# stgl/scarplet

Hardware: AMD Instinct MI355X
Metric: Mpixel·template/s (DEM pixels × ages × orientations / s) (higher is better)
Workload: dtype f32

## Files before the change

scarplet_amd/csrc/sc_api.hip:

```cpp
#include "sc_internal.h"
#include <stdarg.h>
#include <stdio.h>
#include <string.h>
#include <stdlib.h>
#include <math.h>
#include <algorithm>

int sc_fail(sc_ctx* ctx, int code, const char* fmt, ...) {
    char buf[1024];
    va_list ap;
    va_start(ap, fmt);
    vsnprintf(buf, sizeof(buf), fmt, ap);
    va_end(ap);
    if (ctx) ctx->err = buf;
    return code;
}

int sc_ensure(sc_ctx* ctx, DevBuf& b, size_t bytes) {
    if (bytes <= b.cap && b.p) return SC_OK;
    if (b.p) {
        SC_HIP(ctx, hipFree(b.p));
        b.p = nullptr;
        b.cap = 0;
    }
    if (bytes == 0) bytes = 16;
    SC_HIP(ctx, hipMalloc(&b.p, bytes));
    b.cap = bytes;
    return SC_OK;
}

static void buf_free(DevBuf& b) {
    if (b.p) (void)hipFree(b.p);
    b.p = nullptr;
    b.cap = 0;
}

size_t sc_total_bytes(sc_ctx* c) {
    DevBuf* arr[] = {&c->z, &c->xaxis, &c->yaxis, &c->A, &c->B, &c->C, &c->curv,
                     &c->best_snr, &c->best_amp, &c->best_id, &c->map_amp,
                     &c->map_snr, &c->templ, &c->sums, &c->wl1, &c->norms, &c->norm_part, &c->win_w, &c->win_m,
                     &c->tw_y, &c->tw_x, &c->blk, &c->uc, &c->uc2, &c->vh, &c->wh, &c->mh,
                     &c->yw, &c->ym, &c->tiles, &c->halo_z, &c->halo_stage, &c->res, &c->sib_buf, &c->dwin, &c->spans, &c->res_stats, &c->digest, &c->split_s, &c->split_a, &c->split_i,
                     &c->near, &c->near_ev, &c->score, &c->score_w, &c->score_abc, &c->st_slot, &c->st_work, &c->st_pairs, &c->st_patch, &c->st_spans, &c->snap, &c->xch, &c->xch_cnt,
                     &c->tr_planes, &c->tr_thin, &c->tr_par, &c->tr_lab, &c->tr_cnt, &c->tr_bsum, &c->tr_tot, &c->tr_sort, &c->tr_hist, &c->tr_rbsum, &c->tr_seg};
    size_t s = 0;
    for (DevBuf* b : arr) s += b->cap;
    for (auto& w : c->windows) s += (size_t)w.h * w.wd * 13;
    return s;
}

int sc_lds_attr(sc_ctx* ctx, const void* kernel, size_t bytes) {
    auto it = ctx->lds_attr.find(kernel);
    if (it != ctx->lds_attr.end() && it->second >= bytes) return SC_OK;
    SC_HIP(ctx, hipFuncSetAttribute(kernel, hipFuncAttributeMaxDynamicSharedMemorySize,
                                    (int)bytes));
    ctx->lds_attr[kernel] = bytes;
    return SC_OK;
}

void sc_prof_begin(sc_ctx* ctx, int kernel) {
    ctx->prof_cur = -1;
    ctx->prof_kernel = kernel;
    const long long b = ctx->k_brackets[kernel]++;
    if (!ctx->prof) return;
// ... 84 lines not shown
        if (!(value >= 0.0)) return sc_fail(ctx, SC_ERR_INVALID, "batch_fill must be >= 0");
        ctx->batch_fill = (int)value;
    } else if (!strcmp(name, "i1_pairs")) {
        if (!(value >= 1.0 && value <= 64.0)) return sc_fail(ctx, SC_ERR_INVALID, "i1_pairs must be 1 .. 64");
        ctx->i1_pairs = (int)value;
    } else if (!strcmp(name, "near_window")) {
        if (!(value >= 0.0 && value < 1.0)) return sc_fail(ctx, SC_ERR_INVALID, "near_window must be in [0, 1)");
        ctx->near_w = (float)value;
    } else if (!strcmp(name, "batch_templ")) {
        if (!(value >= 0.0 && value <= (double)SC_MAX_BATCH)) return sc_fail(ctx, SC_ERR_INVALID, "batch_templ must be 0 .. %d", SC_MAX_BATCH);
        ctx->batch_templ = (int)value;
    } else if (!strcmp(name, "split_i1")) {
        if (!(value >= 0.0 && value <= 64.0)) return sc_fail(ctx, SC_ERR_INVALID, "split_i1 must be 0 .. 64");
        ctx->split_i1 = (int)value;
    } else if (!strcmp(name, "split_fill")) {
        if (!(value >= 0.0)) return sc_fail(ctx, SC_ERR_INVALID, "split_fill must be >= 0");
        ctx->split_fill = (long long)value;
    } else if (!strcmp(name, "sib")) {
        ctx->sib = (int)value;
    } else if (!strcmp(name, "spectra_mb")) {
        if (!(value >= 0.0)) return sc_fail(ctx, SC_ERR_INVALID, "spectra_mb must be >= 0");
        ctx->spec_mb = value;
        fft_spectra_forget(ctx);
    } else if (!strcmp(name, "y_gb")) {
        if (!(value >= 0.0)) return sc_fail(ctx, SC_ERR_INVALID, "y_gb must be >= 0");
        ctx->y_gb = value;
    } else {
        return sc_fail(ctx, SC_ERR_INVALID, "unknown option '%s'", name);
    }
    return SC_OK;
}

extern "C" int sc_clear_windows(sc_ctx* ctx) {
    if (!ctx) return SC_ERR_INVALID;
    (void)hipStreamSynchronize(ctx->stream);
    for (auto& w : ctx->windows) {
        if (w.w) (void)hipFree(w.w);
        if (w.w64) (void)hipFree(w.w64);
        if (w.m) (void)hipFree(w.m);
        if (w.mask_lim) (void)hipFree(w.mask_lim);
        if (w.mask_err) (void)hipFree(w.mask_err);
    }
    ctx->windows.clear();
    return SC_OK;
}

extern "C" void sc_destroy(sc_ctx* c) {
    if (!c) return;
    (void)hipSetDevice(c->device);
    (void)hipStreamSynchronize(c->stream);
    sc_comm_destroy(c);
    sc_prof_collect(c);
    for (auto& e : c->ev_pool) {
        (void)hipEventDestroy(e.first);
        (void)hipEventDestroy(e.second);
    }
    sc_clear_windows(c);
    DevBuf* arr[] = {&c->z, &c->xaxis, &c->yaxis, &c->A, &c->B, &c->C, &c->curv,
                     &c->best_snr, &c->best_amp, &c->best_id, &c->map_amp,
                     &c->map_snr, &c->templ, &c->sums, &c->wl1, &c->norms, &c->norm_part, &c->win_w, &c->win_m,
                     &c->tw_y, &c->tw_x, &c->blk, &c->uc, &c->uc2, &c->vh, &c->wh, &c->mh,
                     &c->yw, &c->ym, &c->tiles, &c->halo_z, &c->halo_stage, &c->res, &c->sib_buf, &c->dwin, &c->spans, &c->res_stats, &c->digest, &c->split_s, &c->split_a, &c->split_i,
                     &c->near, &c->near_ev, &c->score, &c->score_w, &c->score_abc, &c->st_slot, &c->st_work, &c->st_pairs, &c->st_patch, &c->st_spans, &c->snap, &c->xch, &c->xch_cnt,
                     &c->tr_planes, &c->tr_thin, &c->tr_par, &c->tr_lab, &c->tr_cnt, &c->tr_bsum, &c->tr_tot, &c->tr_sort, &c->tr_hist, &c->tr_rbsum, &c->tr_seg};
    for (DevBuf* b : arr) buf_free(*b);
    for (int k = 0; k < 4; ++k) buf_free(c->cmp[k]);
    for (int k = 0; k < 4; ++k) buf_free(c->cmp_in[k]);
    for (int k = 0; k < 4; ++k) buf_free(c->fill[k]);
    (void)hipStreamDestroy(c->stream);
    delete c;
}

extern "C" const char* sc_last_error(sc_ctx* ctx) {
    return ctx ? ctx->err.c_str() : "null context";
}

extern "C" size_t sc_device_bytes(sc_ctx* ctx) { return ctx ? sc_total_bytes(ctx) : 0; }

static int set_dem_body(sc_ctx* ctx, int ly, int lx, int gy0, int gx0, int ny,
                        int nx, int cy0, int cy1, int cx0, int cx1, double dx,
                        double dy, int wrap, const double* xaxis,
                        const double* yaxis);

static int set_dem_common(sc_ctx* ctx, int ly, int lx, int gy0, int gx0, int ny,
// ... 843 lines not shown
```

scarplet_amd/csrc/sc_fft.hip:

```cpp
#include "sc_internal.h"
#include <math.h>
#include <type_traits>
#include <string.h>

struct TileDev {
    int i0, j0, vy, vx, gi0, gj0;
};

#ifndef SC_I1_XLANE
#define SC_I1_XLANE 1
#endif
#ifndef SC_I2_RD1
#define SC_I2_RD1 1
#endif
#ifndef SC_LDS_WR1
#define SC_LDS_WR1 0
#endif
#ifndef SC_LDS_RD1
#define SC_LDS_RD1 1
#endif
#ifndef SC_H2_XLANE
#define SC_H2_XLANE 1
#endif
#ifndef SC_F1C_HOLD
// ... 1203 lines not shown
    if constexpr (!XP) TAKE_TEMPLATE_SHARE(PT, (size_t)TY * Tx)
    if ((j >> 3) & 1)
        inv_cols_sym_body<TY, true, PT, XP>((Tx >> 2) - 1 - i, uc, uc2, wa, mb, Tx, 0, pair, vfirst, G, rp_lo, rp_hi, phx,
                                            parity, tw, yw, ym, ystride, dbg, np, pcj, tstride, tiles, py_valid);
    else
        inv_cols_sym_body<TY, false, PT, XP>(i, uc, uc2, wa, mb, Tx, 0, pair, vfirst, G, rp_lo, rp_hi, phx,
                                             parity, tw, yw, ym, ystride, dbg, np, pcj, tstride, tiles, py_valid);
}

template <int TY>
__host__ __device__ constexpr int w8_line() { return TY + TY / 16 + 4; }
template <int TY>
__host__ __device__ constexpr size_t w8_lds() {
    return ((size_t)8 * w8_line<TY>() + (SC_I1_TWTAB ? 16 : 4) * (TY / 16 + TY / 256) + SC_MAX_GROUP) * sizeof(float2);
}

template <int TY, bool MIRROR, bool PT, int NC>
__device__ __forceinline__ void
inv_cols_w8_body(const int B, const int jobx, const float2* __restrict__ uc, const float2* __restrict__ uc2,
                 const float* __restrict__ wa, const float* __restrict__ mb, int Tx,
                 int pair, int vfirst, int G, int rp_lo, int rp_hi, const float2* __restrict__ phx,
                 int parity, const float2* __restrict__ tw, float2* __restrict__ yw,
                 float2* __restrict__ ym, int ystride, int np, int pcj, int tstride,
                 const TileDev* __restrict__ tiles, int py_valid, const TemplDev* __restrict__ tl) {
    extern __shared__ __attribute__((aligned(16))) float2 sm[];
    constexpr int S = TY / 16;
    static_assert(S % 64 == 0 && S / 64 <= 2, "one wave per line: 64 or 128 sets");
    constexpr int U = S / 64;
    constexpr int NK = 16 * U;
    constexpr int LINE = w8_line<TY>();
    const int w = __builtin_amdgcn_readfirstlane(threadIdx.x >> 6), lane = threadIdx.x & 63;
    float2* line = sm + w * LINE;
    int i0A = 0, i0B = 0, vyA = 0, vyB = 0;
    {
        const int ob = jobx / pcj, q = jobx - ob * pcj;
        const TileDev tA_ = tiles[2 * (pair + q)], tB_ = tiles[2 * (pair + q) + 1];
        i0A = tA_.i0; i0B = tB_.i0; vyA = tA_.vy; vyB = tB_.vy;
        if (py_valid >= 0) {
            const int vy = max(tA_.vy, tB_.vy);
            rp_hi = min(rp_hi, (py_valid + vy - 1) >> 1);
        }
        pair += ob * np + q;
        vfirst += ob * tstride;
    }
    int2* const rng = reinterpret_cast<int2*>(sm + NC * LINE + (SC_I1_TWTAB ? 16 : 4) * (S + S / 16));
    {
        const int NGt = PT ? (G + 1) / 2 : G;
// ... 33 lines not shown
        float2* t = st2 ? t2 + (i - S) : t1 + i;
        const float2 wb[4] = {tw[e], tw[2 * e], tw[4 * e], tw[8 * e]};
        pk::v2 wk[16];
        twiddle16_expand(wb, wk);
#pragma unroll
        for (int k = 1; k < 16; ++k) t[k * n] = make_float2(wk[k].x, wk[k].y);
    }
#else
    float2* t2 = t1 + 4 * S;
    for (int i = threadIdx.x; i < 4 * S; i += 64 * NC) t1[i] = tw[(i % S) << (i / S)];
    for (int i = threadIdx.x; i < 4 * (S / 16); i += 64 * NC) t2[i] = tw[((i % (S / 16)) << 4) << (i / (S / 16))];
#endif
    auto tw_of = [&](const float2* t, int n, int idx, float2 (&wq)[4]) {
#pragma unroll
        for (int m = 0; m < 4; ++m) wq[m] = lds_cell<true>(t + m * n + idx);
    };
    float c[NK], c2[PT ? NK : 1];
    const int NG = PT ? (G + 1) / 2 : G;
    for (int pl = 0; pl < 2; ++pl) {
        const float2* xcol = (pl ? uc2 : uc) + (size_t)pair * plane + (size_t)ft * TY;
        const float* hsrc = (pl ? mb : wa) + (size_t)vfirst * hplane + (size_t)fs * TY;
        const bool rot = pl == 0 && parity == 1;
        float2 xp[NK];
#pragma unroll
        for (int k = 0; k < NK; ++k) {
            const int fy = lane + 64 * k;
            float2 pv;
            if (!MIRROR) {
                pv = phase_tab(tw + TY, phx, fy, ft);
            } else {
                pv = phase_tab(tw + TY, phx, (TY - fy) & (TY - 1), (Tx - ft) & (Tx - 1));
                pv.y = -pv.y;
            }
            float2 v = cmul(xcol[fy], pv);
            if (rot) v = MIRROR ? make_float2(v.y, -v.x) : make_float2(-v.y, v.x);
            xp[k] = v;
        }
        const float* cbase = hsrc + (MIRROR ? TY - lane : lane);
        const int c0off = (MIRROR && lane == 0) ? -TY : 0;
        auto fetch = [&](int gi_, int u) {
            const float* p = cbase + (size_t)(PT ? 2 * gi_ : gi_) * hplane;
            const bool has2 = PT && 2 * gi_ + 1 < G;
            const float* p2 = has2 ? p + hplane : p;
            const unsigned keep2 = has2 ? ~0u : 0u;
#pragma unroll
            for (int k = 0; k < NK; ++k) {
                if (u >= 0 && k % U != u) continue;
                const int off = k ? (MIRROR ? -64 * k : 64 * k) : c0off;
                c[k] = p[off];
                if constexpr (PT) c2[k] = __uint_as_float(__float_as_uint(p2[off]) & keep2);
            }
        };
        fetch(0, -1);
        for (int gi_ = 0; gi_ < NG; ++gi_) {
            lds_barrier();
            float2 wq[4];
            int lt = lane;
            asm volatile("" : "+v"(lt));
#pragma unroll
// ... 90 lines not shown
                    __builtin_nontemporal_store(f2{c0.x, c0.y}, reinterpret_cast<f2*>(p));
                    __builtin_nontemporal_store(f2{c1.x, c1.y}, reinterpret_cast<f2*>(p + Tx));
                }
            } else
#endif
#pragma unroll 2
            for (int rp = s_lo + RQ * w + ln / NC; rp <= s_hi; rp += RQ * NC)
                store_stream(o + (size_t)rp * (Tx >> 3) * 16, lds_cell<true>(lc + ph(2 * rp)), lds_cell<true>(lc + ph(2 * rp + 1)));
#ifdef SC_I1_PRIO
            __builtin_amdgcn_s_setprio(0);
#endif
        }
        lds_barrier();
    }
}

template <int TY, bool PT>
__global__ void __launch_bounds__(512, (TY == 1024 && !PT) ? 4 : 2)
k_inv_cols_w8(const float2* __restrict__ uc, const float2* __restrict__ uc2,
              const float* __restrict__ wa, const float* __restrict__ mb, int Tx,
              int pair, int vfirst, int G, int rp_lo, int rp_hi, const float2* __restrict__ phx,
              int parity, const float2* __restrict__ tw, float2* __restrict__ yw,
              float2* __restrict__ ym, int ystride, int np, int pcj, int tstride,
              const TileDev* __restrict__ tiles, int py_valid, const TemplDev* __restrict__ tl, int jil) {
    const int L = blockIdx.x, g16 = L / (16 * jil), r16 = L - g16 * 16 * jil, jq = r16 >> 4, j = r16 & 15;
    const int i = (g16 << 3) | (j & 7), jobx = (int)blockIdx.y * jil + jq;
    TAKE_TEMPLATE_SHARE(PT, (size_t)TY * Tx)
    if ((j >> 3) & 1)
        inv_cols_w8_body<TY, true, PT, 8>((Tx >> 3) - 1 - i, jobx, uc, uc2, wa, mb, Tx, pair, vfirst, G, rp_lo,
                                   rp_hi, phx, parity, tw, yw, ym, ystride, np, pcj, tstride, tiles, py_valid, tl);
    else
        inv_cols_w8_body<TY, false, PT, 8>(i, jobx, uc, uc2, wa, mb, Tx, pair, vfirst, G, rp_lo,
                                    rp_hi, phx, parity, tw, yw, ym, ystride, np, pcj, tstride, tiles, py_valid, tl);
}

template <int TY, bool PT>
__global__ void __launch_bounds__(256, 1)
k_inv_cols_w4(const float2* __restrict__ uc, const float2* __restrict__ uc2,
              const float* __restrict__ wa, const float* __restrict__ mb, int Tx,
              int pair, int vfirst, int G, int rp_lo, int rp_hi, const float2* __restrict__ phx,
              int parity, const float2* __restrict__ tw, float2* __restrict__ yw,
              float2* __restrict__ ym, int ystride, int np, int pcj, int tstride,
              const TileDev* __restrict__ tiles, int py_valid, const TemplDev* __restrict__ tl) {
    const int j = blockIdx.x, i = ((j >> 4) << 3) | (j & 7);
    if ((j >> 3) & 1)
        inv_cols_w8_body<TY, true, PT, 4>((Tx >> 2) - 1 - i, (int)blockIdx.y, uc, uc2, wa, mb, Tx, pair, vfirst, G, rp_lo,
                                          rp_hi, phx, parity, tw, yw, ym, ystride, np, pcj, tstride, tiles, py_valid, tl);
    else
        inv_cols_w8_body<TY, false, PT, 4>(i, (int)blockIdx.y, uc, uc2, wa, mb, Tx, pair, vfirst, G, rp_lo,
                                           rp_hi, phx, parity, tw, yw, ym, ystride, np, pcj, tstride, tiles, py_valid, tl);
}

constexpr int H2_TY = 512, H2_COLS = 16;
__host__ __device__ constexpr size_t h2_lds() {
    return ((size_t)H2_COLS * w8_line<H2_TY>() + 4 * (H2_TY / 16 + H2_TY / 256) + SC_MAX_GROUP) * sizeof(float2);
}
template <bool MIRROR, bool PT, bool XP>
__device__ __forceinline__ void
inv_cols_h2_body(const int B, const int jobx, const float2* __restrict__ uc, const float2* __restrict__ uc2,
                 const float* __restrict__ wa, const float* __restrict__ mb, int Tx,
                 int pair, int vfirst, int G, int rp_lo, int rp_hi, const float2* __restrict__ phx,
                 int parity, const float2* __restrict__ tw, float2* __restrict__ yw,
                 float2* __restrict__ ym, int ystride, int np, int pcj, int tstride,
                 const TileDev* __restrict__ tiles, int py_valid, const TemplDev* __restrict__ tl) {
    extern __shared__ __attribute__((aligned(16))) float2 sm[];
    constexpr int TY = H2_TY, S = TY / 16, NK = 16, NC = H2_COLS;
    constexpr int LINE = w8_line<TY>();
    static_assert(S == 32 && !(XP && !PT), "half a wave per column; paired orientations are a paired-template mode");
    const int w = __builtin_amdgcn_readfirstlane(threadIdx.x >> 6), lane = threadIdx.x & 63;
    const int hl = lane & 31, cw = 2 * w + (lane >> 5);
    float2* line = sm + cw * LINE;
    int i0A = 0, i0B = 0, vyA = 0, vyB = 0, pairB = 0;
    if constexpr (XP) {
// ... 1003 lines not shown
}

static int upload_twiddles(sc_ctx* ctx, DevBuf& buf, int& have, int T, int kph) {
    const int key = T * 8 + (kph & 7);
    if (have == key) return SC_OK;
    std::vector<float2> h(2 * (size_t)T);
    for (int k = 0; k < T; ++k) {
        double a = -2.0 * M_PI * (double)k / (double)T;
        h[k] = make_float2((float)cos(a), (float)sin(a));
        long long m = ((long long)kph * k) % (2LL * T);
        double b = M_PI * (double)m / (double)T;
        h[T + k] = make_float2((float)cos(b), (float)sin(b));
    }
    int rc = sc_ensure(ctx, buf, sizeof(float2) * h.size());
    if (rc) return rc;
    SC_HIP(ctx, hipStreamSynchronize(ctx->stream));
    SC_HIP(ctx, hipMemcpy(buf.p, h.data(), sizeof(float2) * h.size(), hipMemcpyHostToDevice));
    have = key;
    return SC_OK;
}

static int npairs_of(const FftGeom& fg) { return (fg.ntiles + 1) / 2; }

void fft_spectra_forget(sc_ctx* ctx) {
    std::fill(ctx->spec_key.begin(), ctx->spec_key.end(), NAN);
}

int fft_prepare(sc_ctx* ctx, const FftGeom& fg, int n_templ_chunk, int group, int nb, int n_slots) {
    if (!fft_size_supported(fg.Ty) || !fft_size_supported(fg.Tx))
        return sc_fail(ctx, SC_ERR_UNSUPPORTED, "FFT tile %dx%d not supported", fg.Ty, fg.Tx);
    int rc;
    if ((rc = upload_twiddles(ctx, ctx->tw_y, ctx->tw_Ty, fg.Ty, 1 - ctx->g.oy))) return rc;
    if ((rc = upload_twiddles(ctx, ctx->tw_x, ctx->tw_Tx, fg.Tx, 1 - ctx->g.ox))) return rc;
    const Geom& g = ctx->g;
    int np = npairs_of(fg);
    std::vector<TileDev> h(2 * np);
    for (int k = 0; k < 2 * np; ++k) {
        TileDev t{0, 0, 0, 0, 0, 0};
        if (k < fg.ntiles) {
            int ty = k / fg.ntx, tx = k % fg.ntx;
            t.i0 = g.cy0 + ty * fg.Vy;
            t.j0 = g.cx0 + tx * fg.Vx;
            t.vy = std::min(fg.Vy, g.cy1 - t.i0);
            t.vx = std::min(fg.Vx, g.cx1 - t.j0);
            t.gi0 = t.i0 + g.oy - fg.Py;
            t.gj0 = t.j0 + g.ox - fg.Qx;
// ... 17 lines not shown
        const Geom& gg = ctx->g;
        const long long sig[24] = {fg.Ty, fg.Tx, fg.Vy, fg.Vx, fg.nty, fg.ntx, fg.circ_y, fg.circ_x, fg.Py, fg.Qx,
                                   gg.ly, gg.lx, gg.gy0, gg.gx0, gg.ny, gg.nx, gg.cy0, gg.cy1, gg.cx0, gg.cx1,
                                   gg.wrap, n_slots, 0, 0};
        bool keep = n_slots > 0 && 2.0 * (double)plane * np * n_slots <= ctx->spec_mb * 1048576.0;
        if (keep) {
            const double add = 2.0 * (double)plane * np * n_slots - (double)(ctx->uc.cap + ctx->uc2.cap);
            size_t free_b = 0, total_b = 0;
            if (add > 0.0 && (hipMemGetInfo(&free_b, &total_b) != hipSuccess || add > 0.25 * (double)free_b))
                keep = false;
        }
        const int slots = keep ? n_slots : 0;
        const size_t have = std::max(nb, slots);
        if (ctx->uc.cap > 2 * plane * np * have + ((size_t)256 << 20)) {
            SC_HIP(ctx, hipStreamSynchronize(ctx->stream));
            for (DevBuf* b : {&ctx->uc, &ctx->uc2}) {
                if (b->p) SC_HIP(ctx, hipFree(b->p));
                b->p = nullptr;
                b->cap = 0;
            }
        }
        const void *p0 = ctx->uc.p, *p1 = ctx->uc2.p, *p2 = ctx->norms.p;
        if ((rc = sc_ensure(ctx, ctx->norms, sizeof(double) * 2 * np * have))) return rc;
        if ((rc = sc_ensure(ctx, ctx->uc, plane * np * have))) return rc;
        if ((rc = sc_ensure(ctx, ctx->uc2, plane * np * have))) return rc;
        if (!keep || slots != ctx->spec_slots || memcmp(sig, ctx->spec_sig, sizeof(sig)) != 0 ||
            p0 != ctx->uc.p || p1 != ctx->uc2.p || p2 != ctx->norms.p) {
            ctx->spec_key.assign((size_t)3 * slots, NAN);
            memcpy(ctx->spec_sig, sig, sizeof(sig));
        }
        ctx->spec_slots = slots;
        ctx->spec_uc_stride = (size_t)np * fg.Ty * fg.Tx;
        ctx->spec_norm_stride = (size_t)2 * np;
        ctx->uc_off = ctx->norms_off = 0;
    }
    if ((rc = sc_ensure(ctx, ctx->norm_part, sizeof(double) * 2 * np * nb * (fg.Ty / 4)))) return rc;
    if ((rc = sc_ensure(ctx, ctx->curv, sizeof(float) * (size_t)ctx->g.ly * ctx->g.lx * nb))) return rc;
    if ((rc = sc_ensure(ctx, ctx->vh, plane * n_templ_chunk))) return rc;
    size_t hplane = half_plane(fg.Ty, fg.Tx) * sizeof(float2);
    if ((rc = sc_ensure(ctx, ctx->wh, hplane * n_templ_chunk))) return rc;
    if ((rc = sc_ensure(ctx, ctx->mh, hplane * n_templ_chunk))) return rc;
    int pb = 1;
    {
        size_t free_b = 0, total_b = 0;
        double budget = 0.0;
        if (hipMemGetInfo(&free_b, &total_b) == hipSuccess)
            budget = std::min(32e9, 0.25 * (double)(free_b + ctx->yw.cap + ctx->ym.cap));
        if (ctx->y_gb > 0.0) budget = ctx->y_gb * 1e9;
// ... 27 lines not shown
    }
    out.slots = (uint32_t*)ctx->sib_buf.p;
    out.base = (++ctx->sib_epoch) << 8;
    return SC_OK;
}

template <typename K>
static int set_lds(sc_ctx* ctx, K kernel, size_t bytes) {
    return sc_lds_attr(ctx, (const void*)kernel, bytes);
}

#define DISPATCH_T(T, FN)                                                     \
    switch (T) {                                                              \
        case 64: FN(64); break;                                               \
        case 128: FN(128); break;                                             \
        case 256: FN(256); break;                                             \
        case 512: FN(512); break;                                             \
        case 1024: FN(1024); break;                                           \
        case 2048: FN(2048); break;                                           \
        case 4096: FN(4096); break;                                           \
        default: return sc_fail(ctx, SC_ERR_UNSUPPORTED, "tile size %d", T);  \
    }

static int launch_fwd_cols(sc_ctx* ctx, const FftGeom& fg, int nplanes,
                           float2* out0, float2* out1, int split2,
                           const TemplDev* templ = nullptr) {
    size_t lds = fft_lds_bytes(fg.Ty);
    dim3 grid(fg.Tx / 4, nplanes);
    sc_prof_begin(ctx, SC_K_FWD_COLS);
#define FN(T)                                                                  \
    {                                                                          \
        int rc = set_lds(ctx, k_fwd_cols<T>, lds);                             \
        if (rc) return rc;                                                     \
        hipLaunchKernelGGL(k_fwd_cols<T>, grid, dim3(fft_threads(T)), lds,     \
                           ctx->stream, (const float2*)ctx->blk.p, fg.Tx,      \
                           (const float2*)ctx->tw_y.p, out0, out1, split2,     \
                           templ);                                             \
    }
    DISPATCH_T(fg.Ty, FN)
#undef FN
    sc_prof_end(ctx);
    SC_HIP(ctx, hipGetLastError());
    return SC_OK;
}

int fft_forward_curv(sc_ctx* ctx, const FftGeom& fg, int nb, const float (*coef)[3]) {
    int np = npairs_of(fg);
    size_t lds = fft_lds_bytes(fg.Tx);
    dim3 grid(fg.Ty / 4 / FWD_ROWS_RBW, np * nb);
    CurvMix mixc;
    memset(&mixc, 0, sizeof(mixc));
    if (coef) {
        if (nb > SC_MAX_ORIENT) return sc_fail(ctx, SC_ERR_INVALID, "curvature batch of %d planes", nb);
        for (int b = 0; b < nb; ++b)
            for (int j = 0; j < 3; ++j) mixc.c[b][j] = coef[b][j];
    }
    sc_prof_begin(ctx, SC_K_FWD_ROWS);
#define FN2(T, MIXV)                                                           \
    {                                                                          \
        int rc = set_lds(ctx, k_fwd_rows_curv<T, MIXV>, lds);                  \
        if (rc) return rc;                                                     \
        hipLaunchKernelGGL((k_fwd_rows_curv<T, MIXV>), grid, dim3(fft_threads(T)), \
                           lds, ctx->stream, (const float*)(MIXV ? ctx->A.p : ctx->curv.p), \
                           (const float*)ctx->B.p, (const float*)ctx->C.p, mixc, \
                           ctx->g, (const TileDev*)ctx->tiles.p, fg.Ty,        \
                           (const float2*)ctx->tw_x.p, (float2*)ctx->blk.p,    \
                           (double*)ctx->norm_part.p, ctx->dbg, np,            \
                           (size_t)ctx->g.ly * ctx->g.lx);                     \
    }
#define FN(T) { if (coef) FN2(T, true) else FN2(T, false) }
    DISPATCH_T(fg.Tx, FN)
#undef FN
#undef FN2
    hipLaunchKernelGGL(k_tile_norms, dim3(np * nb), dim3(64), 0, ctx->stream,
                       (const double*)ctx->norm_part.p, fg.Ty / 4, (double*)ctx->norms.p + ctx->norms_off);
    sc_prof_end(ctx);
    SC_HIP(ctx, hipGetLastError());
    return launch_fwd_cols(ctx, fg, 2 * np * nb, (float2*)ctx->uc.p + ctx->uc_off, (float2*)ctx->uc2.p + ctx->uc_off, 1);
}

static bool fft_use_sym(const sc_ctx* ctx, const FftGeom& fg, int parity) {
    return parity != 0 && fg.Ty <= 2048 && ctx->variant != 8;
}

int fft_forward_templates(sc_ctx* ctx, const FftGeom& fg, int first, int n, int parity) {
    size_t lds = fft_lds_bytes(fg.Tx);
    dim3 grid(fg.Ty / 4, n);
    sc_prof_begin(ctx, SC_K_FWD_ROWS);
#define FN(T)                                                                  \
    {                                                                          \
        int rc = set_lds(ctx, k_fwd_rows_templ<T>, lds);                       \
        if (rc) return rc;                                                     \
        hipLaunchKernelGGL(k_fwd_rows_templ<T>, grid, dim3(fft_threads(T)),    \
                           lds, ctx->stream, (const TemplDev*)ctx->templ.p,    \
                           first, (const float*)ctx->win_w.p,                  \
                           (const uint8_t*)ctx->win_m.p,                       \
                           (const double*)ctx->sums.p, fg.Ty,                  \
                           (const float2*)ctx->tw_x.p, (float2*)ctx->blk.p);   \
    }
    DISPATCH_T(fg.Tx, FN)
#undef FN
// ... 5 lines not shown
        sc_prof_begin(ctx, SC_K_FWD_COLS);
#define FN(T)                                                                  \
    {                                                                          \
        int rc = set_lds(ctx, k_fwd_cols_tsym<T>, ldsc);                       \
        if (rc) return rc;                                                     \
        hipLaunchKernelGGL(k_fwd_cols_tsym<T>, gridc, dim3(fft_threads(T)), ldsc, ctx->stream, \
                           (const float2*)ctx->blk.p, fg.Tx, (const float2*)ctx->tw_y.p, \
                           (const TemplDev*)ctx->templ.p + first, (const float2*)ctx->tw_x.p + fg.Tx, \
                           parity, (float*)ctx->wh.p, (float*)ctx->mh.p);      \
    }
        switch (fg.Ty) {
            case 64: FN(64); break;
            case 128: FN(128); break;
            case 256: FN(256); break;
            case 512: FN(512); break;
            case 1024: FN(1024); break;
            default: FN(2048); break;
        }
#undef FN
        sc_prof_end(ctx);
        SC_HIP(ctx, hipGetLastError());
        return SC_OK;
    }
    int rc = launch_fwd_cols(ctx, fg, n, (float2*)ctx->vh.p, nullptr, 0,
                             (const TemplDev*)ctx->templ.p + first);
    if (rc) return rc;
    size_t cells = half_plane(fg.Ty, fg.Tx);
    dim3 grid_s((unsigned)((cells / 2 + 255) / 256), n);
    sc_prof_begin(ctx, SC_K_FWD_COLS);
    if (fft_use_sym(ctx, fg, parity))
        hipLaunchKernelGGL(k_split_templ_sym, grid_s, dim3(256), 0, ctx->stream,
                           (const float2*)ctx->vh.p, fg.Ty, fg.Tx, (const float2*)ctx->tw_y.p + fg.Ty,
                           (const float2*)ctx->tw_x.p + fg.Tx,
                           parity, (float*)ctx->wh.p, (float*)ctx->mh.p);
    else
        hipLaunchKernelGGL(k_split_templ, grid_s, dim3(256), 0, ctx->stream, (const float2*)ctx->vh.p,
                           fg.Ty, fg.Tx, (float2*)ctx->wh.p, (float2*)ctx->mh.p);
    sc_prof_end(ctx);
    SC_HIP(ctx, hipGetLastError());
    return SC_OK;
}

int fft_inverse_fold(sc_ctx* ctx, const FftGeom& fg, int first, int n,
                     int group, bool to_maps, bool full_masks, int parity, int nb) {
    const bool sym = fft_use_sym(ctx, fg, parity);
    int np = npairs_of(fg);
    size_t lds_r = fft_lds_bytes(fg.Tx);
    int rp_lo = 0, rp_hi = fg.Ty / 2 - 1;
    if (!fg.circ_y) {
        rp_lo = fg.Py / 2;
        rp_hi = std::min(fg.Ty - 1, fg.Py + fg.Vy - 1) / 2;
    }
    const int rp_n = rp_hi - rp_lo + 1;
    if (group > SC_MAX_GROUP)
        return sc_fail(ctx, SC_ERR_INVALID, "group %d exceeds %d", group, SC_MAX_GROUP);
    const int pb = std::max(1, ctx->fft_pb);
    const size_t yblock = (size_t)fg.Ty * fg.Tx * group;
    const bool fast = (fg.Tx == 512 || fg.Tx == 1024 || fg.Tx == 2048) && ctx->variant != 9;
    const bool symx = sym && ctx->variant != 6 && fg.Ty >= 512 && fg.Ty <= 2048 && (fg.Tx / 8) % 8 == 0;
    const bool w8 = symx && ctx->variant != 2 && (fg.Ty == 2048 || fg.Ty == 1024) && (fg.Tx / 16) % 8 == 0;
    if (nb > 1 && (!fast || n > group || nb * n > SC_MAX_BATCH || n > SC_MAX_GROUP))
        return sc_fail(ctx, SC_ERR_INVALID, "orientation batching outside its conditions");
    auto chunk = [&](int pair0, int pc, auto ptc) -> int {
        constexpr bool PTV = decltype(ptc)::value;
        for (int g0 = 0; g0 < n; g0 += group) {
            int G = std::min(group, n - g0);
            const bool xp = PTV && n == 1 && nb >= 2 && pc == 1 && sym && symx && fg.Ty == 512 &&
                            ctx->variant != 12 && !to_maps;
            const size_t lds_c = (size_t)4 * fft_line(fg.Ty) * sizeof(float2) +
                                 (fg.Ty <= 2048 ? (size_t)4 * fg.Ty * sizeof(float2) : 0);
            const int slots = 256 * (int)std::max<size_t>(1, (size_t)(160 * 1024) / lds_c);
            int pi1 = nb > 1 ? pc : std::max(1, std::min(pc, (slots + fg.Tx / 8 - 1) / (fg.Tx / 8)));
            int jil = 1;
            if (nb == 1 && w8 && (!PTV || fg.Ty == 1024) && ctx->variant != 1 && !xp && ctx->i1_pairs > 1) {
                jil = std::min(pc, ctx->i1_pairs);
                pi1 = jil;
            }
            const bool row_skip = !full_masks && !to_maps && ctx->variant != 13;
            auto parts_for = [&](long long workgroups, long long capacity, int transforms) {
                if (!ctx->split_i1 || workgroups <= 0) return 1;
                if (ctx->split_i1 > 1) return std::max(1, std::min(ctx->split_i1, transforms));
                int best = 1;
                double best_u = 0.0;
                for (int nz = 1; nz <= 8 && transforms / nz >= 4; ++nz) {
                    const long long w = workgroups * nz, rounds = (w + capacity - 1) / capacity;
// ... 20 lines not shown
    ctx->stream, (const float2*)ctx->uc.p + ctx->uc_off, (const float2*)ctx->uc2.p + ctx->uc_off, (const float*)ctx->wh.p, \
        (const float*)ctx->mh.p, fg.Tx, CB0, pair, g0, G, rp_lo, rp_hi,                    \
        (const float2*)ctx->tw_x.p + fg.Tx, parity, (const float2*)ctx->tw_y.p, ywp, ymp, group
#define SYM_ARGS_D(CB0) SYM_ARGS(CB0), ctx->dbg, np, pcc, n, (const TileDev*)ctx->tiles.p, fg.circ_y ? -1 : fg.Py
#define FN_SYMX(T)                                                             \
    {                                                                          \
        int rc = set_lds(ctx, k_inv_cols_symx<T, PTV>, inv_cols_lds<T>());     \
        if (rc) return rc;                                                     \
        const int nz_ = parts_for((long long)(fg.Tx / 4) * nb * pcc,                                \
                                  256LL * std::max<size_t>(1, std::min<size_t>((160 * 1024) / inv_cols_lds<T>(), \
                                                                               2048 / fft_threads(T) / 2)), NGl); \
        hipLaunchKernelGGL((k_inv_cols_symx<T, PTV>), dim3(fg.Tx / 4, nb * pcc, nz_), dim3(fft_threads(T)), \
                           inv_cols_lds<T>(), ctx->stream, (const float2*)ctx->uc.p + ctx->uc_off, (const float2*)ctx->uc2.p + ctx->uc_off, \
                           (const float*)ctx->wh.p, (const float*)ctx->mh.p, fg.Tx, pair, g0, G, rp_lo, rp_hi, \
                           (const float2*)ctx->tw_x.p + fg.Tx, parity, (const float2*)ctx->tw_y.p, ywp, ymp, group, \
                           ctx->dbg, np, pcc, n, (const TileDev*)ctx->tiles.p, fg.circ_y ? -1 : fg.Py); \
    }
#define FN_W8(T)                                                               \
    {                                                                          \
        int rc = set_lds(ctx, k_inv_cols_w8<T, PTV>, w8_lds<T>());             \
        if (rc) return rc;                                                     \
        const int nz_ = parts_for((long long)(fg.Tx / 8) * nb * pcc, 256LL * ((T == 1024 && !PTV) ? 2 : 1), NGl); \
        hipLaunchKernelGGL((k_inv_cols_w8<T, PTV>), dim3(fg.Tx / 8 * jilc, nb * pcc / jilc, nz_), dim3(512),  \
                           w8_lds<T>(), ctx->stream, (const float2*)ctx->uc.p + ctx->uc_off, (const float2*)ctx->uc2.p + ctx->uc_off, \
                           (const float*)ctx->wh.p, (const float*)ctx->mh.p, fg.Tx, pair, g0, G, rp_lo, rp_hi, \
                           (const float2*)ctx->tw_x.p + fg.Tx, parity, (const float2*)ctx->tw_y.p, ywp, ymp, group, \
                           np, pcc, n, (const TileDev*)ctx->tiles.p, fg.circ_y ? -1 : fg.Py, \
                           row_skip ? (const TemplDev*)ctx->templ.p + first : nullptr, jilc); \
    }
#define FN_W4(T)                                                               \
    {                                                                          \
         \
        const size_t lds4 = (size_t)88 * 1024;                                 \
        int rc = set_lds(ctx, k_inv_cols_w4<T, PTV>, lds4);                    \
        if (rc) return rc;                                                     \
        hipLaunchKernelGGL((k_inv_cols_w4<T, PTV>), dim3(fg.Tx / 4, nb * pcc), dim3(256),  \
                           lds4, ctx->stream, (const float2*)ctx->uc.p + ctx->uc_off, (const float2*)ctx->uc2.p + ctx->uc_off, \
                           (const float*)ctx->wh.p, (const float*)ctx->mh.p, fg.Tx, pair, g0, G, rp_lo, rp_hi, \
                           (const float2*)ctx->tw_x.p + fg.Tx, parity, (const float2*)ctx->tw_y.p, ywp, ymp, group, \
                           np, pcc, n, (const TileDev*)ctx->tiles.p, fg.circ_y ? -1 : fg.Py, \
                           row_skip ? (const TemplDev*)ctx->templ.p + first : nullptr); \
    }
#define FN_SYM(T)                                                              \
    {                                                                          \
        int rc = set_lds(ctx, k_inv_cols_sym<T, false, PTV>, inv_cols_lds<T>());    \
        if (rc) return rc;                                                     \
        rc = set_lds(ctx, k_inv_cols_sym<T, true, PTV>, inv_cols_lds<T>());         \
        if (rc) return rc;                                                     \
        const int nlo = fg.Tx / 8, nhi = fg.Tx / 4 - nlo;                      \
        hipLaunchKernelGGL((k_inv_cols_sym<T, false, PTV>), dim3(nlo, nb * pcc), dim3(fft_threads(T)), \
                           inv_cols_lds<T>(), SYM_ARGS_D(0));                  \
        if (nhi > 0)                                                           \
            hipLaunchKernelGGL((k_inv_cols_sym<T, true, PTV>), dim3(nhi, nb * pcc), dim3(fft_threads(T)), \
                               inv_cols_lds<T>(), SYM_ARGS_D(nlo));            \
    }
#define FN(T)                                                                  \
    {                                                                          \
        int rc = set_lds(ctx, k_inv_cols<T, false>, inv_cols_lds<T>());        \
        if (rc) return rc;                                                     \
        rc = set_lds(ctx, k_inv_cols<T, true>, inv_cols_lds<T>());             \
        if (rc) return rc;                                                     \
        const int nlo = fg.Tx / 8, nhi = fg.Tx / 4 - nlo;                      \
        hipLaunchKernelGGL((k_inv_cols<T, false>), dim3(nlo, nb * pcc), dim3(fft_threads(T)), \
                           inv_cols_lds<T>(), COL_ARGS(0));                    \
// ... 219 lines not shown
```

scarplet_amd/csrc/sc_internal.h:

```cpp
#pragma once
#include <hip/hip_runtime.h>
#include <stdint.h>
#include <string>
#include <vector>
#include <map>
#include <limits.h>
#include "../../include/scarplet_hip.h"

#define SC_EPS 2.220446049250313e-16
#define SC_EVENT_WORDS 4

#ifdef SC_ABLATE
#define SC_DBGBIT(d, b) (((d) & (b)) != 0)
#else
#define SC_DBGBIT(d, b) false
#endif
#define SC_EXP_UNDERFLOW 745.1332191019412

struct TemplDev {
    int32_t kind, flags;
    double cos_a, sin_a, c, d, p0, p1;
    int32_t ilo, ihi, jlo, jhi;
    int32_t pmin, pmax, qmin, qmax;
    uint32_t id;
// ... 52 lines not shown
    long long dem_nan = 0;
    double dem_sig[16] = {0};
    bool dem_unchanged = false;
    DevBuf digest;
    DevBuf best_snr, best_amp, best_id;
    DevBuf map_amp, map_snr;
    DevBuf cmp[4], cmp_in[4];
    size_t cmp_n = 0;
    DevBuf res_stats;
    DevBuf dwin, spans;
    DevBuf templ, sums, wl1, norms, win_w, win_m;
    DevBuf norm_part;
    double spec_mb = 0.0;
    int spec_slots = 0;
    size_t spec_uc_stride = 0;
    size_t spec_norm_stride = 0;
    size_t uc_off = 0, norms_off = 0;
    std::vector<double> spec_key;
    long long spec_sig[24] = {0};
    DevBuf tw_y, tw_x;
    int tw_Ty = 0, tw_Tx = 0;
    int fft_pb = 1;
    DevBuf blk, uc, uc2, vh, wh, mh, yw, ym, tiles;
    std::vector<WindowSlot> windows;
    std::vector<TemplDev> h_templ;
    std::vector<double> h_sums, h_wl1;
    std::vector<int> h_wslot;
    std::vector<double> h_mix;
    std::vector<unsigned char> h_tiles;
    bool async_in_flight = false;
    int last_batch = 0;
    float kappa = 4.f;
    float near_w = 0.f;
    float near_w_used = 0.f;
    DevBuf near;
    DevBuf near_ev;
    DevBuf st_slot, st_work, st_pairs, st_patch, st_spans;
    DevBuf snap;
    size_t snap_cells = 0;
    long long cand_n = -1;
    DevBuf xch, xch_cnt;
    long long xch_n = -1;
    size_t patch_n = 0;
    DevBuf score;
    DevBuf score_w;
    DevBuf score_abc;
// ... 191 lines not shown
```

Measured before the change: 192,700.

## Fuse forward column FFT of curvature spectra into w8 inverse column kernel

When enabled (default on) and spectra are not cached, the row-FFT output is kept in a new buffer and the forward column FFT is performed inside the w8 inverse-column kernel, loading from that buffer into LDS, instead of running a separate forward-column pass that writes uc/uc2. This removes one full kernel launch and a global round-trip of the spectra. The catch is that the forward column FFT is recomputed in every inverse-column launch (per template group), and the fused kernel carries more registers. A fallback materializes uc/uc2 when the fused path doesn't apply.

Result: faster. 197,400, median of 6 (+2.4%).

```diff
diff --git a/scarplet_amd/csrc/sc_api.hip b/scarplet_amd/csrc/sc_api.hip
--- a/scarplet_amd/csrc/sc_api.hip
+++ b/scarplet_amd/csrc/sc_api.hip
@@ -39,7 +39,7 @@
     DevBuf* arr[] = {&c->z, &c->xaxis, &c->yaxis, &c->A, &c->B, &c->C, &c->curv,
                      &c->best_snr, &c->best_amp, &c->best_id, &c->map_amp,
                      &c->map_snr, &c->templ, &c->sums, &c->wl1, &c->norms, &c->norm_part, &c->win_w, &c->win_m,
-                     &c->tw_y, &c->tw_x, &c->blk, &c->uc, &c->uc2, &c->vh, &c->wh, &c->mh,
+                     &c->tw_y, &c->tw_x, &c->blk, &c->cblk, &c->uc, &c->uc2, &c->vh, &c->wh, &c->mh,
                      &c->yw, &c->ym, &c->tiles, &c->halo_z, &c->halo_stage, &c->res, &c->sib_buf, &c->dwin, &c->spans, &c->res_stats, &c->digest, &c->split_s, &c->split_a, &c->split_i,
                      &c->near, &c->near_ev, &c->score, &c->score_w, &c->score_abc, &c->st_slot, &c->st_work, &c->st_pairs, &c->st_patch, &c->st_spans, &c->snap, &c->xch, &c->xch_cnt,
                      &c->tr_planes, &c->tr_thin, &c->tr_par, &c->tr_lab, &c->tr_cnt, &c->tr_bsum, &c->tr_tot, &c->tr_sort, &c->tr_hist, &c->tr_rbsum, &c->tr_seg};
@@ -170,6 +170,8 @@
         if (!(value >= 0.0)) return sc_fail(ctx, SC_ERR_INVALID, "spectra_mb must be >= 0");
         ctx->spec_mb = value;
         fft_spectra_forget(ctx);
+    } else if (!strcmp(name, "fuse_fwd")) {
+        ctx->fuse_fwd = value != 0.0;
     } else if (!strcmp(name, "y_gb")) {
         if (!(value >= 0.0)) return sc_fail(ctx, SC_ERR_INVALID, "y_gb must be >= 0");
         ctx->y_gb = value;
@@ -207,7 +209,7 @@
     DevBuf* arr[] = {&c->z, &c->xaxis, &c->yaxis, &c->A, &c->B, &c->C, &c->curv,
                      &c->best_snr, &c->best_amp, &c->best_id, &c->map_amp,
                      &c->map_snr, &c->templ, &c->sums, &c->wl1, &c->norms, &c->norm_part, &c->win_w, &c->win_m,
-                     &c->tw_y, &c->tw_x, &c->blk, &c->uc, &c->uc2, &c->vh, &c->wh, &c->mh,
+                     &c->tw_y, &c->tw_x, &c->blk, &c->cblk, &c->uc, &c->uc2, &c->vh, &c->wh, &c->mh,
                      &c->yw, &c->ym, &c->tiles, &c->halo_z, &c->halo_stage, &c->res, &c->sib_buf, &c->dwin, &c->spans, &c->res_stats, &c->digest, &c->split_s, &c->split_a, &c->split_i,
                      &c->near, &c->near_ev, &c->score, &c->score_w, &c->score_abc, &c->st_slot, &c->st_work, &c->st_pairs, &c->st_patch, &c->st_spans, &c->snap, &c->xch, &c->xch_cnt,
                      &c->tr_planes, &c->tr_thin, &c->tr_par, &c->tr_lab, &c->tr_cnt, &c->tr_bsum, &c->tr_tot, &c->tr_sort, &c->tr_hist, &c->tr_rbsum, &c->tr_seg};
diff --git a/scarplet_amd/csrc/sc_fft.hip b/scarplet_amd/csrc/sc_fft.hip
--- a/scarplet_amd/csrc/sc_fft.hip
+++ b/scarplet_amd/csrc/sc_fft.hip
@@ -1249,7 +1249,7 @@
                  int pair, int vfirst, int G, int rp_lo, int rp_hi, const float2* __restrict__ phx,
                  int parity, const float2* __restrict__ tw, float2* __restrict__ yw,
                  float2* __restrict__ ym, int ystride, int np, int pcj, int tstride,
-                 const TileDev* __restrict__ tiles, int py_valid, const TemplDev* __restrict__ tl) {
+                 const TileDev* __restrict__ tiles, int py_valid, const TemplDev* __restrict__ tl, const bool fwd) {
     extern __shared__ __attribute__((aligned(16))) float2 sm[];
     constexpr int S = TY / 16;
     static_assert(S % 64 == 0 && S / 64 <= 2, "one wave per line: 64 or 128 sets");
@@ -1329,19 +1329,108 @@
         const float* hsrc = (pl ? mb : wa) + (size_t)vfirst * hplane + (size_t)fs * TY;
         const bool rot = pl == 0 && parity == 1;
         float2 xp[NK];
-#pragma unroll
-        for (int k = 0; k < NK; ++k) {
-            const int fy = lane + 64 * k;
-            float2 pv;
-            if (!MIRROR) {
-                pv = phase_tab(tw + TY, phx, fy, ft);
+        auto park = [&](auto get) {
+#pragma unroll
+            for (int k = 0; k < NK; ++k) {
+                const int fy = lane + 64 * k;
+                float2 pv;
+                if (!MIRROR) {
+                    pv = phase_tab(tw + TY, phx, fy, ft);
+                } else {
+                    pv = phase_tab(tw + TY, phx, (TY - fy) & (TY - 1), (Tx - ft) & (Tx - 1));
+                    pv.y = -pv.y;
+                }
+                float2 v = cmul(get(k), pv);
+                if (rot) v = MIRROR ? make_float2(v.y, -v.x) : make_float2(-v.y, v.x);
+                xp[k] = v;
+            }
+        };
+        if (fwd) {
+            constexpr int CH = 4 * NC;
+            constexpr int EP = TY / 128;
+            {
+                int tid = threadIdx.x;
+                asm volatile("" : "+v"(tid));
+                const int i = (2 * tid) % CH, rb = (2 * tid) / CH;
+                const float2* src = uc + (size_t)(2 * pair + pl) * plane + (size_t)B * CH + (size_t)rb * (Tx >> 2) * 16 + i;
+                const size_t step = (size_t)32 * (Tx >> 2) * 16;
+                float2* dst = sm + (4 * (i >> 4) + (i & 3)) * LINE + ph(4 * rb + ((i >> 2) & 3));
+                float4 x[EP];
+#pragma unroll
+                for (int u = 0; u < EP; ++u) x[u] = *reinterpret_cast<const float4*>(src + u * step);
+#pragma unroll
+                for (int u = 0; u < EP; ++u) {
+                    dst[u * 136] = make_float2(x[u].x, x[u].y);
+                    dst[u * 136 + LINE] = make_float2(x[u].z, x[u].w);
+                }
+            }
+            lds_barrier();
+            int lt = lane;
+            asm volatile("" : "+v"(lt));
+            float2 wq[4];
+            float2 a[U][16];
+#pragma unroll
+            for (int u = 0; u < U; ++u) set_load<TY, true>(line, lt + 64 * u, a[u]);
+            asm volatile("" ::: "memory");
+#pragma unroll
+            for (int u = 0; u < U; ++u) {
+#if SC_I1_TWTAB
+                set_compute_store<TY, 16, 0, false, true>(line, lt + 64 * u, a[u], wq, t1 + lt + 64 * u, S);
+#else
+                tw_of(t1, S, lt + 64 * u, wq);
+                set_compute_store<TY, 16, 0, false, false, true>(line, lt + 64 * u, a[u], wq);
+#endif
+            }
+            asm volatile("" ::: "memory");
+#pragma unroll
+            for (int u = 0; u < U; ++u) set_load<TY, true>(line, lt + 64 * u, a[u]);
+            if constexpr (SC_I1_XLANE) {
+                float2 o2[U][16];
+#pragma unroll
+                for (int u = 0; u < U; ++u) {
+#if SC_I1_TWTAB
+                    set_compute_regs<false, true>(a[u], wq, o2[u], t2 + ((lt + 64 * u) >> 4), S / 16);
+#else
+                    tw_of(t2, S / 16, (lt + 64 * u) >> 4, wq);
+                    set_compute_regs<false>(a[u], wq, o2[u]);
+#endif
+                }
+#pragma unroll
+                for (int u = 0; u < U; ++u)
+#pragma unroll
+                    for (int mh = 0; mh < 4; ++mh) {
+                        xlane_transpose4(o2[u][4 * mh].x, o2[u][4 * mh + 1].x, o2[u][4 * mh + 2].x, o2[u][4 * mh + 3].x);
+                        xlane_transpose4(o2[u][4 * mh].y, o2[u][4 * mh + 1].y, o2[u][4 * mh + 2].y, o2[u][4 * mh + 3].y);
+                    }
+                constexpr int R3x = TY / 256, NB3 = 16 / R3x;
+#pragma unroll
+                for (int u3 = 0; u3 < U; ++u3)
+#pragma unroll
+                    for (int b = 0; b < NB3; ++b)
+#pragma unroll
+                        for (int j = 0; j < R3x; ++j) a[u3][b + NB3 * j] = o2[j >> 2][4 * (u3 + U * b) + (j & 3)];
             } else {
-                pv = phase_tab(tw + TY, phx, (TY - fy) & (TY - 1), (Tx - ft) & (Tx - 1));
-                pv.y = -pv.y;
-            }
-            float2 v = cmul(xcol[fy], pv);
-            if (rot) v = MIRROR ? make_float2(v.y, -v.x) : make_float2(-v.y, v.x);
-            xp[k] = v;
+                asm volatile("" ::: "memory");
+#pragma unroll
+                for (int u = 0; u < U; ++u) {
+#if SC_I1_TWTAB
+                    set_compute_store<TY, 16, 4, false, true>(line, lt + 64 * u, a[u], wq, t2 + ((lt + 64 * u) >> 4), S / 16);
+#else
+                    tw_of(t2, S / 16, (lt + 64 * u) >> 4, wq);
+                    set_compute_store<TY, 16, 4, false, false, true>(line, lt + 64 * u, a[u], wq);
+#endif
+                }
+                asm volatile("" ::: "memory");
+#pragma unroll
+                for (int u = 0; u < U; ++u) set_load<TY, true>(line, lt + 64 * u, a[u]);
+                asm volatile("" ::: "memory");
+            }
+#pragma unroll
+            for (int u = 0; u < U; ++u) set_compute_store<TY, TY / 256, 8, false, false, true>(line, lt + 64 * u, a[u], wq);
+            asm volatile("" ::: "memory");
+            park([&](int k) { return lds_cell<true>(line + ph(lt + 64 * k)); });
+        } else {
+            park([&](int k) { return xcol[lane + 64 * k]; });
         }
         const float* cbase = hsrc + (MIRROR ? TY - lane : lane);
         const int c0off = (MIRROR && lane == 0) ? -TY : 0;
@@ -1478,16 +1567,16 @@
               int pair, int vfirst, int G, int rp_lo, int rp_hi, const float2* __restrict__ phx,
               int parity, const float2* __restrict__ tw, float2* __restrict__ yw,
               float2* __restrict__ ym, int ystride, int np, int pcj, int tstride,
-              const TileDev* __restrict__ tiles, int py_valid, const TemplDev* __restrict__ tl, int jil) {
+              const TileDev* __restrict__ tiles, int py_valid, const TemplDev* __restrict__ tl, int jil, int fwd) {
     const int L = blockIdx.x, g16 = L / (16 * jil), r16 = L - g16 * 16 * jil, jq = r16 >> 4, j = r16 & 15;
     const int i = (g16 << 3) | (j & 7), jobx = (int)blockIdx.y * jil + jq;
     TAKE_TEMPLATE_SHARE(PT, (size_t)TY * Tx)
     if ((j >> 3) & 1)
         inv_cols_w8_body<TY, true, PT, 8>((Tx >> 3) - 1 - i, jobx, uc, uc2, wa, mb, Tx, pair, vfirst, G, rp_lo,
-                                   rp_hi, phx, parity, tw, yw, ym, ystride, np, pcj, tstride, tiles, py_valid, tl);
+                                   rp_hi, phx, parity, tw, yw, ym, ystride, np, pcj, tstride, tiles, py_valid, tl, fwd != 0);
     else
         inv_cols_w8_body<TY, false, PT, 8>(i, jobx, uc, uc2, wa, mb, Tx, pair, vfirst, G, rp_lo,
-                                    rp_hi, phx, parity, tw, yw, ym, ystride, np, pcj, tstride, tiles, py_valid, tl);
+                                    rp_hi, phx, parity, tw, yw, ym, ystride, np, pcj, tstride, tiles, py_valid, tl, fwd != 0);
 }
 
 template <int TY, bool PT>
@@ -1497,14 +1586,14 @@
               int pair, int vfirst, int G, int rp_lo, int rp_hi, const float2* __restrict__ phx,
               int parity, const float2* __restrict__ tw, float2* __restrict__ yw,
               float2* __restrict__ ym, int ystride, int np, int pcj, int tstride,
-              const TileDev* __restrict__ tiles, int py_valid, const TemplDev* __restrict__ tl) {
+              const TileDev* __restrict__ tiles, int py_valid, const TemplDev* __restrict__ tl, int fwd) {
     const int j = blockIdx.x, i = ((j >> 4) << 3) | (j & 7);
     if ((j >> 3) & 1)
         inv_cols_w8_body<TY, true, PT, 4>((Tx >> 2) - 1 - i, (int)blockIdx.y, uc, uc2, wa, mb, Tx, pair, vfirst, G, rp_lo,
-                                          rp_hi, phx, parity, tw, yw, ym, ystride, np, pcj, tstride, tiles, py_valid, tl);
+                                          rp_hi, phx, parity, tw, yw, ym, ystride, np, pcj, tstride, tiles, py_valid, tl, fwd != 0);
     else
         inv_cols_w8_body<TY, false, PT, 4>(i, (int)blockIdx.y, uc, uc2, wa, mb, Tx, pair, vfirst, G, rp_lo,
-                                           rp_hi, phx, parity, tw, yw, ym, ystride, np, pcj, tstride, tiles, py_valid, tl);
+                                           rp_hi, phx, parity, tw, yw, ym, ystride, np, pcj, tstride, tiles, py_valid, tl, fwd != 0);
 }
 
 constexpr int H2_TY = 512, H2_COLS = 16;
@@ -2554,6 +2643,11 @@
 
 static int npairs_of(const FftGeom& fg) { return (fg.ntiles + 1) / 2; }
 
+static bool fft_fuse_curv(const sc_ctx* ctx, const FftGeom& fg, int slots) {
+    return ctx->fuse_fwd && slots == 0 && (fg.Ty == 2048 || fg.Ty == 1024) && (fg.Tx / 16) % 8 == 0 &&
+           ctx->variant != 1 && ctx->variant != 2 && ctx->variant != 6 && ctx->variant != 8;
+}
+
 void fft_spectra_forget(sc_ctx* ctx) {
     std::fill(ctx->spec_key.begin(), ctx->spec_key.end(), NAN);
 }
@@ -2617,8 +2711,13 @@
         }
         const void *p0 = ctx->uc.p, *p1 = ctx->uc2.p, *p2 = ctx->norms.p;
         if ((rc = sc_ensure(ctx, ctx->norms, sizeof(double) * 2 * np * have))) return rc;
-        if ((rc = sc_ensure(ctx, ctx->uc, plane * np * have))) return rc;
-        if ((rc = sc_ensure(ctx, ctx->uc2, plane * np * have))) return rc;
+        if (fft_fuse_curv(ctx, fg, slots)) {
+            if ((rc = sc_ensure(ctx, ctx->cblk, plane * 2 * np * nb))) return rc;
+        } else {
+            if ((rc = sc_ensure(ctx, ctx->uc, plane * np * have))) return rc;
+            if ((rc = sc_ensure(ctx, ctx->uc2, plane * np * have))) return rc;
+        }
+        ctx->curv_rows = 0;
         if (!keep || slots != ctx->spec_slots || memcmp(sig, ctx->spec_sig, sizeof(sig)) != 0 ||
             p0 != ctx->uc.p || p1 != ctx->uc2.p || p2 != ctx->norms.p) {
             ctx->spec_key.assign((size_t)3 * slots, NAN);
@@ -2692,7 +2791,7 @@
         default: return sc_fail(ctx, SC_ERR_UNSUPPORTED, "tile size %d", T);  \
     }
 
-static int launch_fwd_cols(sc_ctx* ctx, const FftGeom& fg, int nplanes,
+static int launch_fwd_cols(sc_ctx* ctx, const FftGeom& fg, const float2* in, int nplanes,
                            float2* out0, float2* out1, int split2,
                            const TemplDev* templ = nullptr) {
     size_t lds = fft_lds_bytes(fg.Ty);
@@ -2703,7 +2802,7 @@
         int rc = set_lds(ctx, k_fwd_cols<T>, lds);                             \
         if (rc) return rc;                                                     \
         hipLaunchKernelGGL(k_fwd_cols<T>, grid, dim3(fft_threads(T)), lds,     \
-                           ctx->stream, (const float2*)ctx->blk.p, fg.Tx,      \
+                           ctx->stream, in, fg.Tx,                             \
                            (const float2*)ctx->tw_y.p, out0, out1, split2,     \
                            templ);                                             \
     }
@@ -2718,6 +2817,8 @@
     int np = npairs_of(fg);
     size_t lds = fft_lds_bytes(fg.Tx);
     dim3 grid(fg.Ty / 4 / FWD_ROWS_RBW, np * nb);
+    const bool fuse = fft_fuse_curv(ctx, fg, ctx->spec_slots);
+    float2* rows_out = (float2*)(fuse ? ctx->cblk.p : ctx->blk.p);
     CurvMix mixc;
     memset(&mixc, 0, sizeof(mixc));
     if (coef) {
@@ -2734,7 +2835,7 @@
                            lds, ctx->stream, (const float*)(MIXV ? ctx->A.p : ctx->curv.p), \
                            (const float*)ctx->B.p, (const float*)ctx->C.p, mixc, \
                            ctx->g, (const TileDev*)ctx->tiles.p, fg.Ty,        \
-                           (const float2*)ctx->tw_x.p, (float2*)ctx->blk.p,    \
+                           (const float2*)ctx->tw_x.p, rows_out,               \
                            (double*)ctx->norm_part.p, ctx->dbg, np,            \
                            (size_t)ctx->g.ly * ctx->g.lx);                     \
     }
@@ -2746,7 +2847,9 @@
                        (const double*)ctx->norm_part.p, fg.Ty / 4, (double*)ctx->norms.p + ctx->norms_off);
     sc_prof_end(ctx);
     SC_HIP(ctx, hipGetLastError());
-    return launch_fwd_cols(ctx, fg, 2 * np * nb, (float2*)ctx->uc.p + ctx->uc_off, (float2*)ctx->uc2.p + ctx->uc_off, 1);
+    ctx->curv_rows = fuse ? 2 * np * nb : 0;
+    if (fuse) return SC_OK;
+    return launch_fwd_cols(ctx, fg, rows_out, 2 * np * nb, (float2*)ctx->uc.p + ctx->uc_off, (float2*)ctx->uc2.p + ctx->uc_off, 1);
 }
 
 static bool fft_use_sym(const sc_ctx* ctx, const FftGeom& fg, int parity) {
@@ -2798,7 +2901,7 @@
         SC_HIP(ctx, hipGetLastError());
         return SC_OK;
     }
-    int rc = launch_fwd_cols(ctx, fg, n, (float2*)ctx->vh.p, nullptr, 0,
+    int rc = launch_fwd_cols(ctx, fg, (const float2*)ctx->blk.p, n, (float2*)ctx->vh.p, nullptr, 0,
                              (const TemplDev*)ctx->templ.p + first);
     if (rc) return rc;
     size_t cells = half_plane(fg.Ty, fg.Tx);
@@ -2837,6 +2940,19 @@
     const bool w8 = symx && ctx->variant != 2 && (fg.Ty == 2048 || fg.Ty == 1024) && (fg.Tx / 16) % 8 == 0;
     if (nb > 1 && (!fast || n > group || nb * n > SC_MAX_BATCH || n > SC_MAX_GROUP))
         return sc_fail(ctx, SC_ERR_INVALID, "orientation batching outside its conditions");
+    const bool fwd = ctx->curv_rows > 0 && w8 && ctx->variant != 1 && !to_maps;
+    if (ctx->curv_rows > 0 && !fwd) {
+        const size_t half = (size_t)fg.Ty * fg.Tx * sizeof(float2) * (ctx->curv_rows / 2);
+        int rc;
+        if ((rc = sc_ensure(ctx, ctx->uc, half))) return rc;
+        if ((rc = sc_ensure(ctx, ctx->uc2, half))) return rc;
+        if ((rc = launch_fwd_cols(ctx, fg, (const float2*)ctx->cblk.p, ctx->curv_rows, (float2*)ctx->uc.p + ctx->uc_off,
+                                  (float2*)ctx->uc2.p + ctx->uc_off, 1)))
+            return rc;
+        ctx->curv_rows = 0;
+    }
+    const float2* const xc = fwd ? (const float2*)ctx->cblk.p : (const float2*)ctx->uc.p + ctx->uc_off;
+    const float2* const xc2 = fwd ? (const float2*)ctx->cblk.p : (const float2*)ctx->uc2.p + ctx->uc_off;
     auto chunk = [&](int pair0, int pc, auto ptc) -> int {
         constexpr bool PTV = decltype(ptc)::value;
         for (int g0 = 0; g0 < n; g0 += group) {
@@ -2903,11 +3019,11 @@
         if (rc) return rc;                                                     \
         const int nz_ = parts_for((long long)(fg.Tx / 8) * nb * pcc, 256LL * ((T == 1024 && !PTV) ? 2 : 1), NGl); \
         hipLaunchKernelGGL((k_inv_cols_w8<T, PTV>), dim3(fg.Tx / 8 * jilc, nb * pcc / jilc, nz_), dim3(512),  \
-                           w8_lds<T>(), ctx->stream, (const float2*)ctx->uc.p + ctx->uc_off, (const float2*)ctx->uc2.p + ctx->uc_off, \
+                           w8_lds<T>(), ctx->stream, xc, xc2, \
                            (const float*)ctx->wh.p, (const float*)ctx->mh.p, fg.Tx, pair, g0, G, rp_lo, rp_hi, \
                            (const float2*)ctx->tw_x.p + fg.Tx, parity, (const float2*)ctx->tw_y.p, ywp, ymp, group, \
                            np, pcc, n, (const TileDev*)ctx->tiles.p, fg.circ_y ? -1 : fg.Py, \
-                           row_skip ? (const TemplDev*)ctx->templ.p + first : nullptr, jilc); \
+                           row_skip ? (const TemplDev*)ctx->templ.p + first : nullptr, jilc, fwd ? 1 : 0); \
     }
 #define FN_W4(T)                                                               \
     {                                                                          \
@@ -2916,11 +3032,11 @@
         int rc = set_lds(ctx, k_inv_cols_w4<T, PTV>, lds4);                    \
         if (rc) return rc;                                                     \
         hipLaunchKernelGGL((k_inv_cols_w4<T, PTV>), dim3(fg.Tx / 4, nb * pcc), dim3(256),  \
-                           lds4, ctx->stream, (const float2*)ctx->uc.p + ctx->uc_off, (const float2*)ctx->uc2.p + ctx->uc_off, \
+                           lds4, ctx->stream, xc, xc2, \
                            (const float*)ctx->wh.p, (const float*)ctx->mh.p, fg.Tx, pair, g0, G, rp_lo, rp_hi, \
                            (const float2*)ctx->tw_x.p + fg.Tx, parity, (const float2*)ctx->tw_y.p, ywp, ymp, group, \
                            np, pcc, n, (const TileDev*)ctx->tiles.p, fg.circ_y ? -1 : fg.Py, \
-                           row_skip ? (const TemplDev*)ctx->templ.p + first : nullptr); \
+                           row_skip ? (const TemplDev*)ctx->templ.p + first : nullptr, fwd ? 1 : 0); \
     }
 #define FN_SYM(T)                                                              \
     {                                                                          \
diff --git a/scarplet_amd/csrc/sc_internal.h b/scarplet_amd/csrc/sc_internal.h
--- a/scarplet_amd/csrc/sc_internal.h
+++ b/scarplet_amd/csrc/sc_internal.h
@@ -98,6 +98,9 @@
     int tw_Ty = 0, tw_Tx = 0;
     int fft_pb = 1;
     DevBuf blk, uc, uc2, vh, wh, mh, yw, ym, tiles;
+    int fuse_fwd = 1;
+    DevBuf cblk;
+    int curv_rows = 0;
     std::vector<WindowSlot> windows;
     std::vector<TemplDev> h_templ;
     std::vector<double> h_sums, h_wl1;
```
